# AiX-im/Sample-based-GNN

Measured on AMD Instinct MI355X. Metric: sampled-edges/sec + epoch time, 2-hop GCN on Reddit-shaped graph @1/2/4/8 GPUs, higher is better.
Workload: dtype fp32 (GEMM inputs fp32, split exactly into three bf16 pieces in the kernels, 6 bf16 MFMA products, fp32 accumulate; aggregation fp32)

## Files before the change

sample-based-gnn_amd/csrc/common.hpp:

```cpp
#pragma once
#include <hip/hip_runtime.h>

#include <algorithm>
#include <cstdint>
#include <cstdio>
#include <cstring>
#include <string>
#include <utility>
#include <vector>

#include "nts_hip.h"

namespace nts_hip {

void set_error(const char* fmt, ...);
bool launch_trace();
void launch_trace_sync(const char* file, int line);

#define NTS_HIP_TRY(expr)                                                        \
  do {                                                                           \
    hipError_t _e = (expr);                                                      \
    if (_e != hipSuccess) {                                                      \
      ::nts_hip::set_error("%s:%d: %s failed: %s", __FILE__, __LINE__, #expr,    \
                           hipGetErrorString(_e));                               \
// ... 179 lines not shown
                       __HIP_MEMORY_SCOPE_AGENT);
  return prefix;
}

struct CountArgs {
  const uint64_t* goff;
  const uint32_t* dst;
  const uint32_t* v_in;
  uint32_t v_cap;
  int fanout;
  uint32_t* sizes;
  uint32_t e_cap;
  const uint32_t* omit_map;
  uint32_t omit_key;
  const uint32_t* omit_loc;
  uint32_t* omit_row;
};
int count_scan(nts_hip_ctx* ctx, const CountArgs& ca, uint32_t* co, hipStream_t stream);
size_t count_scan_tmp_elems(uint64_t v_cap);

int radix_sort_pairs(const uint32_t* keys_in, const uint32_t* vals_in, uint32_t* keys_out,
                     uint32_t* vals_out, const uint32_t* n_dev, uint64_t n_cap,
                     uint32_t bits, void* tmp, hipStream_t stream, nts_hip_ctx* ctx = nullptr);
size_t radix_tmp_bytes(uint64_t n_cap);
struct RadixPayload {
  const uint32_t* p1_in = nullptr;
  uint32_t* p1_out = nullptr;
  const uint32_t* p2_in = nullptr;
  uint32_t* p2_out = nullptr;
};
int radix_pass_pairs(const uint32_t* keys_in, const uint32_t* vals_in, uint32_t* keys_out,
                     uint32_t* vals_out, const uint32_t* n_dev, uint64_t n_cap, uint32_t shift,
                     uint32_t dbits, void* tmp, hipStream_t stream, const uint32_t** totals,
                     const RadixPayload& pl = RadixPayload{});
size_t radix_pass_tmp_bytes(uint64_t n_cap);

int sum_splits(hipStream_t st, const float* part, int splits, uint64_t stride, int M, int N,
               float* C, uint64_t ldc);

bool gemm3_nn_ok(int M, int N, int K, const float* A, uint64_t lda);
bool gemm3_tn_ok(int M, int N, int K);
int gemm3_nn(nts_hip_ctx* ctx, bool epi, int M, int N, int K, const float* A, uint64_t lda,
             const uint32_t* amap, const float* B, uint64_t ldb, float* C, uint64_t ldc,
             uint32_t keep_threshold, float scale, uint64_t seed, uint64_t offset);
int gemm3_tn(nts_hip_ctx* ctx, int M, int N, int K, const float* A, uint64_t lda,
             const uint32_t* amap, const float* B, uint64_t ldb, const float* X, uint64_t ldx,
             float bscale, float* C, uint64_t ldc);
bool x3_tn_ok(int M, int N, int K, const float* A, uint64_t lda, const float* B, uint64_t ldb,
              const float* Xm = nullptr, uint64_t ldxm = 0);
bool x3_tn_bm_ok(int M, int N, int K, const float* A, uint64_t lda, const float* B, uint64_t ldb,
                 const float* Xm, uint64_t ldxm);
int x3_tn(nts_hip_ctx* ctx, int M, int N, int K, const float* A, uint64_t lda, const uint32_t* amap,
          const float* B, uint64_t ldb, float* C, uint64_t ldc, const float* Xm = nullptr,
          uint64_t ldxm = 0, float bscale = 1.f);
bool x3_nn_ok(int M, int N, int K, const float* A, uint64_t lda);
bool x3_nn7_ok(int M, int N, int K, const float* A, uint64_t lda);
bool x3_nnk_ok(int M, int N, int K, const float* A, uint64_t lda);
int x3_nn(nts_hip_ctx* ctx, bool epi, int M, int N, int K, const float* A, uint64_t lda,
          const uint32_t* amap, const char* bimg, float* C, uint64_t ldc, uint32_t keep_threshold,
          float scale, uint64_t seed, uint64_t offset);
}
```

sample-based-gnn_amd/csrc/primitives.hip:

```cpp
#include "common.hpp"
#include "radix_tile.hpp"

namespace nts_hip {

constexpr int kScanThreads = 256;
constexpr int kScanItems = 16;
constexpr int kScanTile = kScanThreads * kScanItems;

__device__ __forceinline__ uint32_t pad_idx(uint32_t j) { return j + (j >> 4); }

template <typename T>
__device__ __forceinline__ T wave_incl_scan(T x, int lane) {
#pragma unroll
  for (int o = 1; o < kWave; o <<= 1) {
    T y = __shfl_up(x, o, kWave);
    if (lane >= o) x += y;
  }
  return x;
}

template <typename T>
__device__ __forceinline__ T block_excl_scan(T x, T* wsum , T* total) {
  const int t = threadIdx.x, lane = t & 63, w = t >> 6;
  T inc = wave_incl_scan(x, lane);
// ... 296 lines not shown
  NTS_RET(ensure_scan_state(ctx, scan1_state_elems(n_cap)));
  hipLaunchKernelGGL((k_scan1<false, kScanItems>), dim3((uint32_t)nb), dim3(kScanThreads), 0, stream, in, out,
                     n_dev, n_cap, ctx->scan_state, next_epoch(ctx), scan_ticket(ctx), CountArgs{});
  NTS_LAUNCH_CHECK();
  return NTS_OK;
}

size_t count_scan_tmp_elems(uint64_t v_cap) { return scan_tmp_elems<uint32_t>(v_cap) + 64; }

int count_scan(nts_hip_ctx* ctx, const CountArgs& ca, uint32_t* co, hipStream_t stream) {
  constexpr int kCountItems = 4;
  const uint64_t nb = (uint64_t)ca.v_cap / (kScanThreads * kCountItems) + 1;
  NTS_RET(ensure_scan_state(ctx, (nb + 63) / 64 * 64));
  hipLaunchKernelGGL((k_scan1<true, kCountItems>), dim3((uint32_t)nb), dim3(kScanThreads), 0, stream, nullptr,
                     co, nullptr, (uint64_t)ca.v_cap, ctx->scan_state, next_epoch(ctx), scan_ticket(ctx), ca);
  NTS_LAUNCH_CHECK();
  return NTS_OK;
}

template int scan_exclusive<uint32_t>(const uint32_t*, uint32_t*, const uint32_t*, uint64_t,
                                      uint32_t*, hipStream_t);
template int scan_exclusive<uint64_t>(const uint64_t*, uint64_t*, const uint32_t*, uint64_t,
                                      uint64_t*, hipStream_t);
template size_t scan_tmp_elems<uint32_t>(uint64_t);
template size_t scan_tmp_elems<uint64_t>(uint64_t);

template <int IT>
__global__ __launch_bounds__(kRadixThreads) void k_radix_hist(const uint32_t* __restrict__ keys,
                                                              const uint32_t* n_dev,
                                                              uint64_t n_cap, uint32_t shift,
                                                              uint32_t mask, uint32_t* hist,
                                                              uint32_t nb) {
  __shared__ uint32_t h[kRadixMaxBins];
  const int t = threadIdx.x;
  const uint32_t bins = mask + 1;
  for (uint32_t d = t; d < bins; d += kRadixThreads) h[d] = 0;
  __syncthreads();
  const uint64_t n = n_dev ? (uint64_t)*n_dev : n_cap;
  const uint64_t base = (uint64_t)blockIdx.x * (kRadixThreads * IT);
  if (base >= n) return;
#pragma unroll
  for (int k = 0; k < IT; ++k) {
    const uint64_t i = base + (uint64_t)k * kRadixThreads + t;
    if (i < n) atomicAdd(&h[(keys[i] >> shift) & mask], 1u);
  }
  __syncthreads();
  for (uint32_t d = t; d < bins; d += kRadixThreads) hist[(uint64_t)d * nb + blockIdx.x] = h[d];
}

__global__ __launch_bounds__(kRadixThreads) void k_radix_rowscan(uint32_t* __restrict__ hist,
                                                                 const uint32_t* n_dev, uint64_t n_cap,
                                                                 uint32_t nb, uint32_t tile,
                                                                 uint32_t* __restrict__ totals) {
  __shared__ uint32_t wsum[kRadixThreads / kWave];
  const int t = threadIdx.x;
  const uint64_t n = n_dev ? (uint64_t)*n_dev : n_cap;
  const uint32_t live = (uint32_t)((n + tile - 1) / tile);
  uint32_t* row = hist + (uint64_t)blockIdx.x * nb;
  constexpr int kPer = 4;
  uint32_t carry = 0;
  for (uint32_t c0 = 0; c0 < live; c0 += kRadixThreads * kPer) {
    uint32_t v[kPer], sum = 0;
#pragma unroll
    for (int k = 0; k < kPer; ++k) {
      const uint32_t j = c0 + t * kPer + k;
      v[k] = j < live ? row[j] : 0u;
      sum += v[k];
    }
    uint32_t tot;
    uint32_t run = carry + block_excl_scan(sum, wsum, &tot);
#pragma unroll
    for (int k = 0; k < kPer; ++k) {
      const uint32_t j = c0 + t * kPer + k;
      if (j < live) row[j] = run;
      run += v[k];
    }
    carry += tot;
    __syncthreads();
  }
  if (t == 0) totals[blockIdx.x] = carry;
// ... 42 lines not shown
    }
    __syncthreads();
#pragma unroll
    for (int k = 0; k < IT; ++k)
      if (wbase + (uint64_t)k * kWave + lane < n) sm.sv[loc[k]] = pv[k];
    __syncthreads();
    for (uint32_t i = threadIdx.x; i < cnt; i += kRadixThreads)
      pout[radix_tile_pos(sm, i, sm.sk[i], shift, mask)] = sm.sv[i];
  };
  if (p1_out) payload(p1_in, p1_out);
  if (p2_out) payload(p2_in, p2_out);
}

static size_t radix_tmp_bytes_t(uint64_t n_cap, uint32_t tile) {
  uint64_t nb = (n_cap + tile - 1) / tile;
  if (nb == 0) nb = 1;
  size_t hist = (size_t)kRadixMaxBins * nb + 1;
  size_t elems = 2 * ((n_cap + 63) / 64 * 64) + (hist + 63) / 64 * 64 + kRadixMaxBins + 64;
  return elems * sizeof(uint32_t);
}

size_t radix_tmp_bytes(uint64_t n_cap) { return radix_tmp_bytes_t(n_cap, kRadixTile); }
size_t radix_pass_tmp_bytes(uint64_t n_cap) { return radix_tmp_bytes_t(n_cap, kRadixThreads * kRadixPassItems); }

static uint32_t* radix_totals(void* tmp, uint64_t n_cap, uint32_t tile) {
  const uint32_t nb = ceil_div(n_cap, tile);
  const uint64_t n_al = (n_cap + 63) / 64 * 64;
  return (uint32_t*)tmp + 2 * n_al + ((uint64_t)kRadixMaxBins * nb + 1 + 63) / 64 * 64;
}

template <int IT>
static void radix_pass(const uint32_t* ksrc, const uint32_t* vsrc, uint32_t* kdst, uint32_t* vdst,
                       const uint32_t* n_dev, uint64_t n_cap, uint32_t shift, uint32_t dbits,
                       void* tmp, hipStream_t stream, const RadixPayload& pl = RadixPayload{}) {
  constexpr uint32_t tile = kRadixThreads * IT;
  const uint32_t nb = ceil_div(n_cap, tile);
  const uint64_t n_al = (n_cap + 63) / 64 * 64;
  uint32_t* hist = (uint32_t*)tmp + 2 * n_al;
  uint32_t* totals = radix_totals(tmp, n_cap, tile);
  const uint32_t mask = (1u << dbits) - 1u;
  hipLaunchKernelGGL(k_radix_hist<IT>, dim3(nb), dim3(kRadixThreads), 0, stream, ksrc, n_dev, n_cap,
                     shift, mask, hist, nb);
  hipLaunchKernelGGL(k_radix_rowscan, dim3(mask + 1), dim3(kRadixThreads), 0, stream, hist, n_dev,
                     n_cap, nb, tile, totals);
  hipLaunchKernelGGL(k_radix_scatter<IT>, dim3(nb), dim3(kRadixThreads), 0, stream, ksrc, vsrc, kdst,
                     vdst, n_dev, n_cap, shift, dbits, (const uint32_t*)hist, nb,
                     (const uint32_t*)totals, pl.p1_in, pl.p1_out, pl.p2_in, pl.p2_out);
}

int radix_sort_pairs(const uint32_t* keys_in, const uint32_t* vals_in, uint32_t* keys_out,
                     uint32_t* vals_out, const uint32_t* n_dev, uint64_t n_cap, uint32_t bits,
                     void* tmp, hipStream_t stream, nts_hip_ctx* ctx) {
  (void)ctx;
  if (n_cap == 0) return NTS_OK;
  const uint64_t n_al = (n_cap + 63) / 64 * 64;
  uint32_t* ktmp = (uint32_t*)tmp;
  uint32_t* vtmp = ktmp + n_al;
  if (bits < 1) bits = 1;
  const int npass = (int)((bits + kRadixMaxBits - 1) / kRadixMaxBits);
  const uint32_t dbits = (bits + npass - 1) / npass;
  const uint32_t* ksrc = keys_in;
  const uint32_t* vsrc = vals_in;
  for (int p = 0; p < npass; ++p) {
    bool to_out = ((npass - 1 - p) % 2) == 0;
    uint32_t* kdst = to_out ? keys_out : ktmp;
    uint32_t* vdst = to_out ? vals_out : vtmp;
    radix_pass<kRadixItems>(ksrc, vsrc, kdst, vdst, n_dev, n_cap, dbits * p, dbits, tmp, stream);
    NTS_LAUNCH_CHECK();
    ksrc = kdst;
    vsrc = vdst;
  }
  return NTS_OK;
}

int radix_pass_pairs(const uint32_t* keys_in, const uint32_t* vals_in, uint32_t* keys_out,
                     uint32_t* vals_out, const uint32_t* n_dev, uint64_t n_cap, uint32_t shift,
                     uint32_t dbits, void* tmp, hipStream_t stream, const uint32_t** totals,
                     const RadixPayload& pl) {
  NTS_CHECK_ARG(dbits >= 1 && dbits <= (uint32_t)kRadixMaxBits, "radix digit of 1..9 bits");
  NTS_CHECK_ARG(n_cap > 0, "empty capacity");
  NTS_CHECK_ARG(!(pl.p1_out || pl.p2_out) || !vals_in, "payloads need index values (vals_in NULL)");
  radix_pass<kRadixPassItems>(keys_in, vals_in, keys_out, vals_out, n_dev, n_cap, shift, dbits, tmp,
                              stream, pl);
  NTS_LAUNCH_CHECK();
  *totals = radix_totals(tmp, n_cap, kRadixThreads * kRadixPassItems);
  return NTS_OK;
}

}
```

sample-based-gnn_amd/csrc/radix_tile.hpp:

```cpp
#pragma once
#include "common.hpp"

namespace nts_hip {

constexpr int kRadixThreads = 256;
constexpr int kRadixItems = 16;
constexpr int kRadixTile = kRadixThreads * kRadixItems;
constexpr int kRadixPassItems = 4;
constexpr int kRadixMaxBits = 9;
constexpr int kRadixMaxBins = 1 << kRadixMaxBits;

template <int IT>
struct RadixTileLds {
  uint32_t wh[kRadixThreads / kWave][kRadixMaxBins];
  uint32_t gstart[kRadixMaxBins];
  uint32_t lstart[kRadixMaxBins];
  uint32_t sk[kRadixThreads * IT], sv[kRadixThreads * IT];
  uint32_t wsum[kRadixThreads / kWave];
};

template <int IT, class Pub, class GS>
__device__ __forceinline__ void radix_tile_order(RadixTileLds<IT>& sm, const uint32_t* __restrict__ keys_in,
                                                 const uint32_t* __restrict__ vals_in, uint64_t n,
                                                 uint32_t shift, uint32_t dbits, Pub&& publish,
                                                 GS&& gstart, uint32_t (&loc)[IT]) {
  const int t = threadIdx.x, lane = t & 63, w = t >> 6;
  const uint64_t base = (uint64_t)blockIdx.x * (kRadixThreads * IT);
  const uint32_t mask = (1u << dbits) - 1u, bins = mask + 1;
  for (uint32_t d = t; d < bins; d += kRadixThreads)
#pragma unroll
    for (int ww = 0; ww < kRadixThreads / kWave; ++ww) sm.wh[ww][d] = 0;
  __syncthreads();
  const uint64_t lt_mask = (lane == 0) ? 0ull : (~0ull >> (64 - lane));
  const uint64_t wbase = base + (uint64_t)w * (IT * kWave);
  uint32_t key[IT], val[IT], rank[IT];
#pragma unroll
  for (int k = 0; k < IT; ++k) {
    const uint64_t i = wbase + (uint64_t)k * kWave + lane;
    const bool valid = i < n;
    key[k] = valid ? keys_in[i] : 0u;
    val[k] = valid ? (vals_in ? vals_in[i] : (uint32_t)i) : 0u;
  }
#pragma unroll
  for (int k = 0; k < IT; ++k) {
    const bool valid = wbase + (uint64_t)k * kWave + lane < n;
    const uint32_t d = (key[k] >> shift) & mask;
    uint64_t peers = __ballot(valid);
    for (uint32_t b = 0; b < dbits; ++b) {
      const bool bit = (d >> b) & 1u;
      const uint64_t m = __ballot(bit);
      peers &= bit ? m : ~m;
    }
// ... 66 lines not shown
```

sample-based-gnn_amd/csrc/sampler.hip:

```cpp
#include "mfma_lds.hpp"

#include <type_traits>

namespace nts_hip {

constexpr int kSelThreads = 256;
constexpr int kSelWaves = kSelThreads / kWave;
constexpr int kSetCap = 1024;

__device__ __forceinline__ uint32_t philox_word(uint64_t seed, uint32_t dst, uint32_t layer,
                                                uint64_t batch_seq, uint32_t idx) {
  uint4 c = make_uint4(idx >> 2, dst, layer, (uint32_t)batch_seq);
  uint2 k = make_uint2((uint32_t)seed, (uint32_t)(seed >> 32) ^ (uint32_t)(batch_seq >> 32));
  uint4 r = philox4x32_10(c, k);
  uint32_t j = idx & 3u;
  return j == 0 ? r.x : (j == 1 ? r.y : (j == 2 ? r.z : r.w));
}

struct Draw {
  uint32_t range, thr, scaling, past;
  bool lemire;
  __device__ __forceinline__ void init(uint32_t r, bool lem) {
    range = r;
    lemire = lem;
    thr = (0u - r) % r;
    scaling = 0xFFFFFFFFu / r;
    past = r * scaling;
  }
  __device__ __forceinline__ bool apply(uint32_t x, uint32_t& v) const {
    if (lemire) {
      uint64_t m = (uint64_t)x * range;
      v = (uint32_t)(m >> 32);
      return (uint32_t)m >= thr;
    }
    v = x / scaling;
    return x < past;
  }
};

struct SelectArgs {
  const uint64_t* goff;
  const uint32_t* grows;
  const uint32_t* dst;
  const uint32_t* co;
  uint32_t* sizes;
  uint32_t* ans;
  uint32_t* edst;
  uint8_t* marks;
  uint32_t e_cap;
  int fanout;
  uint32_t layer;
  uint64_t batch_seq;
  uint64_t seed;
};

__device__ __forceinline__ void copy_all(const SelectArgs& a, uint32_t i, uint64_t beg,
                                         uint32_t deg, uint32_t c, int lane) {
  for (uint32_t k = lane; k < deg; k += kWave) {
    uint32_t g = a.grows[beg + k];
    a.ans[c + k] = g;
    a.edst[c + k] = i;
    a.marks[g] = 1;
  }
}

template <typename WordFn>
__device__ __forceinline__ uint32_t select_distinct(const SelectArgs& a, uint32_t i,
                                                    uint64_t beg, uint32_t deg, uint32_t need,
                                                    uint32_t c, int lane, uint32_t* set,
                                                    const Draw& dr, WordFn word) {
  const uint64_t lt_mask = (lane == 0) ? 0ull : (~0ull >> (64 - lane));
  uint32_t count = 0, consumed = 0;
  while (count < need) {
    const uint32_t remaining = need - count;
    const int R = remaining <= 12 ? 16 : (remaining <= 28 ? 32 : 64);
    uint32_t val = 0;
    bool ok = false;
    if (lane < R) ok = dr.apply(word(consumed + lane), val);
    bool dup = false;
    for (uint32_t j = 0; j < count; ++j) dup |= (set[j] == val);
    const uint64_t okmask = __ballot(ok);
// ... 75 lines not shown
      dup |= (j < lane) && ((okmask >> j) & 1ull) && (vj == val);
    }
    const uint64_t newmask = __ballot(ok && !dup);
    uint64_t take = newmask;
    if ((uint32_t)__popcll(newmask) >= remaining) {
      uint64_t m = newmask;
      for (uint32_t t = 1; t < remaining; ++t) m &= m - 1;
      const int last = __ffsll((long long)m) - 1;
      take = newmask & ((last == 63) ? ~0ull : ((2ull << last) - 1ull));
      consumed += (uint32_t)last + 1u;
    } else {
      consumed += (uint32_t)kWave;
    }
    if ((take >> lane) & 1ull) {
      hset_put(hset, mask, val);
      out[count + (uint32_t)__popcll(take & lt_mask)] = val;
    }
    count += (uint32_t)__popcll(take);
    __syncthreads();
  }
  for (uint32_t k = lane; k < cap; k += kWave) hset[k] = 0u;
  __syncthreads();
  return consumed;
}

__global__ __launch_bounds__(kWave) void k_select_philox_big(SelectArgs a, uint32_t cap) {
  extern __shared__ uint32_t hset[];
  const int lane = threadIdx.x;
  for (uint32_t k = lane; k < cap; k += kWave) hset[k] = 0u;
  __syncthreads();
  const uint32_t v = a.sizes[0];
  for (uint32_t i = blockIdx.x; i < v; i += gridDim.x) {
    const uint32_t d = a.dst[i];
    const uint64_t beg = a.goff[d];
    const uint32_t deg = (uint32_t)(a.goff[d + 1] - beg);
    const uint32_t c = a.co[i];
    const uint32_t n = a.co[i + 1] - c;
    if (c + n > a.e_cap) continue;
    if (n == deg) {
      copy_all(a, i, beg, deg, c, lane);
      continue;
    }
    if (n == 0) continue;
    const uint64_t seed = a.seed, bs = a.batch_seq;
    const uint32_t layer = a.layer;
    select_distinct_hashed(n, hset, cap, lane, deg, (0u - deg) % deg, true, a.ans + c,
                           [&](uint32_t j) { return philox_word(seed, d, layer, bs, j); });
    for (uint32_t k = lane; k < n; k += kWave) {
      const uint32_t g = a.grows[beg + a.ans[c + k]];
      a.ans[c + k] = g;
      a.edst[c + k] = i;
      a.marks[g] = 1;
    }
  }
}

__global__ __launch_bounds__(kSelThreads) void k_select_philox(SelectArgs a) {
  __shared__ uint32_t sets[kSelWaves][kSetCap];
  const int lane = threadIdx.x & 63, w = threadIdx.x >> 6;
  const uint32_t v = a.sizes[0];
  uint32_t* set = sets[w];
  const uint32_t nw = gridDim.x * kSelWaves;
  for (uint32_t i = blockIdx.x * kSelWaves + w; i < v; i += nw) {
    const uint32_t d = a.dst[i];
    const uint64_t beg = a.goff[d];
    const uint32_t deg = (uint32_t)(a.goff[d + 1] - beg);
    const uint32_t c = a.co[i];
    const uint32_t n = a.co[i + 1] - c;
    if (c + n > a.e_cap) continue;
    if (n == deg) {
      copy_all(a, i, beg, deg, c, lane);
    } else if (n > 0) {
      Draw dr;
      dr.init(deg, true);
      const uint64_t seed = a.seed;
      const uint32_t layer = a.layer;
      const uint64_t bs = a.batch_seq;
      select_distinct(a, i, beg, deg, n, c, lane, set, dr, [&](uint32_t j) {
        return philox_word(seed, d, layer, bs, j);
      });
    }
  }
}

constexpr int kGrp = 16;
constexpr int kGrpPerWave = kWave / kGrp;

template <int J>
struct GrpDupScan {
  static __device__ __forceinline__ void run(bool& dup, uint32_t val, int gl, uint32_t okm) {
    const uint32_t vj = (uint32_t)__builtin_amdgcn_update_dpp(0, (int)val, 0x150 + J, 0xF, 0xF, false);
    dup |= (J < gl) && ((okm >> J) & 1u) && (vj == val);
    GrpDupScan<J + 1>::run(dup, val, gl, okm);
  }
};
template <>
struct GrpDupScan<kGrp> {
  static __device__ __forceinline__ void run(bool&, uint32_t, int, uint32_t) {}
};

__global__ __launch_bounds__(kSelThreads) void k_select_philox_g16(SelectArgs a) {
  __shared__ uint32_t sets[kSelWaves * kGrpPerWave][kGrp];
  const int lane = threadIdx.x & 63, w = threadIdx.x >> 6;
  const int gl = lane & (kGrp - 1), grp = lane >> 4;
  const int gib = w * kGrpPerWave + grp;
  uint32_t* set = sets[gib];
  const uint32_t gshift = kGrp * grp;
  const uint32_t lt16 = (1u << gl) - 1u;
  const uint32_t v = a.sizes[0];
  const uint32_t ng = gridDim.x * kSelWaves * kGrpPerWave;
  for (uint32_t i = blockIdx.x * kSelWaves * kGrpPerWave + gib; i < v; i += ng) {
    const uint32_t d = a.dst[i];
    const uint64_t beg = a.goff[d];
    const uint32_t deg = (uint32_t)(a.goff[d + 1] - beg);
    const uint32_t c = a.co[i];
    const uint32_t n = a.co[i + 1] - c;
    if (c + n > a.e_cap) continue;
    if (n == deg) {
      for (uint32_t k = gl; k < deg; k += kGrp) {
        const uint32_t g = a.grows[beg + k];
        a.ans[c + k] = g;
        a.edst[c + k] = i;
        a.marks[g] = 1;
      }
      continue;
    }
    if (n == 0) continue;
    Draw dr;
    dr.init(deg, true);
    uint32_t count = 0, consumed = 0;
    while (count < n) {
      const uint32_t remaining = n - count;
      uint32_t val = 0;
      const bool ok = dr.apply(philox_word(a.seed, d, a.layer, a.batch_seq, consumed + gl), val);
      bool dup = false;
      for (uint32_t j = 0; j < count; ++j) dup |= (set[j] == val);
      const uint32_t okm = (uint32_t)(__ballot(ok) >> gshift) & 0xFFFFu;
      GrpDupScan<0>::run(dup, val, gl, okm);
      const bool isnew = ok && !dup;
      const uint32_t newm = (uint32_t)(__ballot(isnew) >> gshift) & 0xFFFFu;
      uint32_t take = newm;
      if ((uint32_t)__popc(newm) >= remaining) {
        uint32_t m = newm;
        for (uint32_t t = 1; t < remaining; ++t) m &= m - 1;
        const int last = __ffs(m) - 1;
// ... 908 lines not shown
  const uint32_t words[4] = {m.x, m.y, m.z, m.w};
  const uint64_t v0 = tid * 16;
#pragma unroll
  for (int q = 0; q < 4; ++q) {
#pragma unroll
    for (int b = 0; b < 4; ++b) {
      if ((words[q] >> (8 * b)) & 0xffu) {
        const uint64_t vtx = v0 + q * 4 + b;
        if (vtx < n_vertices && pos < s_cap) {
          source[pos] = (uint32_t)vtx;
          src_index[vtx] = pos;
        }
        ++pos;
      }
    }
  }
}


struct RelabelArgs {
  const uint32_t* ans;
  const uint32_t* edst;
  const uint32_t* dst;
  const uint32_t* src_index;
  const uint32_t* out_deg;
  const uint32_t* in_deg;
  const uint32_t* co;
  const uint32_t* sizes;
  int weight_type;
  uint32_t* ri;
  float* wf;
  uint32_t* up_cnt;
  uint32_t* pub;
};

__device__ __forceinline__ void publish_sizes(const uint32_t* sizes, uint32_t* pub) {
  if (pub && blockIdx.x == 0 && threadIdx.x < 4) pub[threadIdx.x] = sizes[threadIdx.x];
}

__device__ __forceinline__ uint32_t relabel_one(const RelabelArgs& a, uint32_t k) {
  const uint32_t g = a.ans[k];
  const uint32_t r = a.src_index[g];
  a.ri[k] = r;
  if (a.up_cnt) {
    atomicAdd(a.up_cnt + r, 1u);
  } else if (a.weight_type != NTS_WEIGHT_NONE) {
    const uint32_t dg = a.dst[a.edst[k]];
    const uint32_t ind = a.in_deg[dg];
    float w = norm_degree(a.out_deg[g], ind);
    if (a.weight_type == NTS_WEIGHT_MEAN) w = mean_weight(w, ind);
    if (a.weight_type == NTS_WEIGHT_MEAN_SAMPLED) w = w / (float)(a.co[a.edst[k] + 1] - a.co[a.edst[k]]);
    a.wf[k] = w;
  }
  return r;
}

__global__ void k_relabel(RelabelArgs a) {
  publish_sizes(a.sizes, a.pub);
  const uint32_t e = a.sizes[1];
  for (uint32_t k = blockIdx.x * blockDim.x + threadIdx.x; k < e; k += gridDim.x * blockDim.x)
    relabel_one(a, k);
}

__global__ void k_up_weight(const uint32_t* __restrict__ ri, const uint32_t* __restrict__ edst,
                            const uint32_t* __restrict__ co, const uint32_t* __restrict__ cnt,
                            const uint32_t* sizes, int weight_type, float* __restrict__ wf,
                            uint32_t* pub) {
  publish_sizes(sizes, pub);
  const uint32_t e = sizes[1];
  for (uint32_t k = blockIdx.x * blockDim.x + threadIdx.x; k < e; k += gridDim.x * blockDim.x) {
    const uint32_t d = edst[k];
    const uint32_t ind = co[d + 1] - co[d];
    float w = norm_degree(cnt[ri[k]], ind);
    if (weight_type == NTS_WEIGHT_MEAN || weight_type == NTS_WEIGHT_MEAN_SAMPLED)
      w = w / (float)ind;
    wf[k] = w;
  }
}

__global__ void k_mark_dst(const uint32_t* __restrict__ dst, const uint32_t* sizes,
                           uint8_t* __restrict__ marks) {
  const uint32_t v = sizes[0];
  for (uint32_t d = blockIdx.x * blockDim.x + threadIdx.x; d < v; d += gridDim.x * blockDim.x)
    marks[dst[d]] = 1;
}
__global__ void k_dst_local(const uint32_t* __restrict__ dst, const uint32_t* __restrict__ src_index,
                            const uint32_t* sizes, uint32_t* __restrict__ dl) {
  const uint32_t v = sizes[0];
  for (uint32_t d = blockIdx.x * blockDim.x + threadIdx.x; d < v; d += gridDim.x * blockDim.x)
    dl[d] = src_index[dst[d]];
}

constexpr int kCsrBucketThreads = 1024;
constexpr int kCsrBucketWaves = kCsrBucketThreads / kWave;
constexpr int kCsrBucketIt = 4;

template <int L>
__global__ __launch_bounds__(kCsrBucketThreads) void k_csr_bucket(
    const uint32_t* __restrict__ skey, const uint32_t* __restrict__ seid,
    const uint32_t* __restrict__ totals, const uint32_t* __restrict__ sdst,
    const uint32_t* __restrict__ swf, const uint32_t* sizes, uint32_t* __restrict__ ro,
    uint32_t* __restrict__ ci, float* __restrict__ wb, uint32_t* __restrict__ ceid, uint32_t* pub) {
  constexpr uint32_t R = 1u << L, RPT = R > kCsrBucketThreads ? R / kCsrBucketThreads : 1;
  __shared__ uint32_t wh[kCsrBucketWaves][R];
  __shared__ uint32_t wsum[kCsrBucketWaves];
  publish_sizes(sizes, pub);
  const int t = threadIdx.x, lane = t & 63, w = t >> 6;
  const uint32_t b = blockIdx.x, s = sizes[2], r0 = b << L;
  if (r0 > s) return;
  uint32_t part = 0;
  for (uint32_t i = t; i < b; i += kCsrBucketThreads) part += totals[i];
#pragma unroll
  for (int o = 32; o >= 1; o >>= 1) part += __shfl_xor(part, o, kWave);
  if (lane == 0) wsum[w] = part;
  for (uint32_t d = t; d < R; d += kCsrBucketThreads)
#pragma unroll
    for (int ww = 0; ww < kCsrBucketWaves; ++ww) wh[ww][d] = 0;
  __syncthreads();
  uint32_t bstart = 0;
#pragma unroll
  for (int ww = 0; ww < kCsrBucketWaves; ++ww) bstart += wsum[ww];
  const uint32_t cnt = totals[b];
  const uint32_t q0 = (uint32_t)((uint64_t)cnt * w / kCsrBucketWaves);
// ... 347 lines not shown
  uint32_t* t_swf = t_sdst + sort_p / 2;
  uint32_t* t_up = t_sdst + sort_p;
  uint32_t* t_mt = t_up + up_n;
  void* t_sort = (void*)(t_mt + mt_n);

  const uint32_t gv = std::max(1u, std::min(ceil_div(o->v_cap, 256), kMaxGrid));
  const uint32_t ge = std::max(1u, std::min(ceil_div(o->e_cap, 256), kMaxGrid));

  {
    CountArgs ca;
    ca.goff = g->column_offset;
    ca.dst = o->destination;
    ca.v_in = o->v_size;
    ca.v_cap = o->v_cap;
    ca.fanout = fanout;
    ca.sizes = o->sizes;
    ca.e_cap = o->e_cap;
    ca.omit_map = o->omit_map;
    ca.omit_key = o->omit_key;
    ca.omit_loc = o->omit_loc;
    ca.omit_row = o->omit_row;
    NTS_RET(count_scan(ctx, ca, o->column_offset, st));
  }

  SelectArgs a;
  a.goff = g->column_offset;
  a.grows = g->row_indices;
  a.dst = o->destination;
  a.co = o->column_offset;
  a.sizes = o->sizes;
  a.ans = o->sample_ans;
  a.edst = o->edge_dst;
  a.marks = ctx->marks;
  a.e_cap = o->e_cap;
  a.fanout = fanout;
  a.layer = (uint32_t)layer;
  a.batch_seq = batch_seq;
  a.seed = ctx->seed;
  if (rng_mode == NTS_RNG_PHILOX) {
    if (fanout >= 0 && fanout <= kGrp) {
      const uint32_t gs =
          std::max(1u, std::min(ceil_div(o->v_cap, kSelWaves * kGrpPerWave), 4096u));
      hipLaunchKernelGGL(k_select_philox_g16, dim3(gs), dim3(kSelThreads), 0, st, a);
    } else if (fanout < 0 || fanout <= kSetCap) {
      const uint32_t gs = std::max(1u, std::min(ceil_div(o->v_cap, kSelWaves), 4096u));
      hipLaunchKernelGGL(k_select_philox, dim3(gs), dim3(kSelThreads), 0, st, a);
    } else {
      uint32_t cap = 1;
      while (cap < 2u * (uint32_t)fanout) cap <<= 1;
      const size_t lds = (size_t)cap * sizeof(uint32_t);
      NTS_HIP_TRY(hipFuncSetAttribute(reinterpret_cast<const void*>(&k_select_philox_big),
                                      hipFuncAttributeMaxDynamicSharedMemorySize, (int)lds));
      const uint32_t gs = std::max(1u, std::min(o->v_cap, 2048u));
      hipLaunchKernelGGL(k_select_philox_big, dim3(gs), dim3(kWave), lds, st, a, cap);
    }
  } else {
    const int lem = rng_mode == NTS_RNG_MT19937_LEMIRE ? 1 : 0;
    constexpr int mt_dbg = 0;
    uint4* info = reinterpret_cast<uint4*>(t_mt);
    uint64_t gen_hi = 0;
    uint32_t seq = 0;
    NTS_RET(mt_ring_prepare(ctx, w_cap, st, &gen_hi, &seq));
    if (mt_chunked) {
      uint32_t* base = t_mt + mt_info_n;
      float2* cstat = reinterpret_cast<float2*>(base + mt_base_n);
      uint2* win = reinterpret_cast<uint2*>(base + mt_base_n + mt_stat_n);
// ... 30 lines not shown
      else if (fanout <= 16) NTS_RET(run(I16{}, I16{}));
      else if (fanout <= 25) NTS_RET(run(std::integral_constant<int, 25>{}, I32{}));
      else NTS_RET(run(I32{}, I32{}));
      NTS_LAUNCH_CHECK();
      NTS_RET(mt_ring_finish(ctx, st));
      const uint32_t gs = std::max(1u, std::min(ceil_div(o->v_cap, kSelWaves * kGrpPerWave), 4096u));
      hipLaunchKernelGGL(k_mt_rows, dim3(gs), dim3(kSelThreads), 0, st, a);
      NTS_LAUNCH_CHECK();
      goto frontier;
    }
    hipLaunchKernelGGL(k_mt_prep, dim3(gv), dim3(256), 0, st, g->column_offset, o->destination,
                       o->column_offset, o->sizes, o->e_cap, lem, info, nullptr, nullptr, 1u,
                       nullptr, nullptr);
    NTS_LAUNCH_CHECK();
    const MtChunked whole{ctx->mt_ring, nullptr, gen_hi, nullptr, nullptr, ctx->mt_done, seq,
                          o->sizes + 3};
    if (fanout >= 0 && fanout <= 16)
      hipLaunchKernelGGL((k_mt_serial<16, false>), dim3(1), dim3(kWave), 0, st, info, o->sizes,
                         o->sample_ans, ctx->mt_state, lem, mt_dbg, whole);
    else if (fanout >= 0 && fanout <= 32)
      hipLaunchKernelGGL((k_mt_serial<32, false>), dim3(1), dim3(kWave), 0, st, info, o->sizes,
                         o->sample_ans, ctx->mt_state, lem, mt_dbg, whole);
    else
      hipLaunchKernelGGL((k_mt_serial<64, false>), dim3(1), dim3(kWave), 0, st, info, o->sizes,
                         o->sample_ans, ctx->mt_state, lem, mt_dbg, whole);
    NTS_LAUNCH_CHECK();
    NTS_RET(mt_ring_finish(ctx, st));
    const uint32_t gs = std::max(1u, std::min(ceil_div(o->v_cap, kSelWaves * kGrpPerWave), 4096u));
    hipLaunchKernelGGL(k_mt_rows, dim3(gs), dim3(kSelThreads), 0, st, a);
  }
  NTS_LAUNCH_CHECK();

frontier:
  if (o->dst_local_id) {
    hipLaunchKernelGGL(k_mark_dst, dim3(gv), dim3(256), 0, st, o->destination, o->sizes,
                       ctx->marks);
    NTS_LAUNCH_CHECK();
  }

  constexpr uint32_t kMarkFusedMaxTiles = 256;
  if (nblk_marks <= kMarkFusedMaxTiles) {
    NTS_RET(ensure_scan_state(ctx, scan1_state_elems((uint64_t)nblk_marks * 4096)));
    hipLaunchKernelGGL(k_mark_fused, dim3(nblk_marks), dim3(kMarkThreads), 0, st, ctx->marks,
                       nblk_marks, V, o->s_cap, o->source, ctx->src_index, o->sizes,
                       ctx->scan_state, scan_next_epoch(ctx), scan_ticket(ctx));
    NTS_LAUNCH_CHECK();
  } else {
    hipLaunchKernelGGL(k_mark_count, dim3(nblk_marks), dim3(kMarkThreads), 0, st, ctx->marks,
                       t_blk);
    NTS_LAUNCH_CHECK();
    if (nblk_marks <= kMarkDirectTiles) {
      hipLaunchKernelGGL(k_mark_write<true>, dim3(nblk_marks), dim3(kMarkThreads), 0, st,
                         ctx->marks, t_blk, nblk_marks, V, o->s_cap, o->source, ctx->src_index,
                         o->sizes);
    } else {
      NTS_RET(scan_exclusive<uint32_t>(t_blk, t_blk, nullptr, nblk_marks, t_scan_blk, st));
      hipLaunchKernelGGL(k_mark_write<false>, dim3(nblk_marks), dim3(kMarkThreads), 0, st,
                         ctx->marks, t_blk, nblk_marks, V, o->s_cap, o->source, ctx->src_index,
                         o->sizes);
    }
    NTS_LAUNCH_CHECK();
  }

  if (o->dst_local_id) {
    hipLaunchKernelGGL(k_dst_local, dim3(gv), dim3(256), 0, st, o->destination, ctx->src_index,
                       o->sizes, o->dst_local_id);
    NTS_LAUNCH_CHECK();
  }

  RelabelArgs ra{o->sample_ans,      o->edge_dst, o->destination, ctx->src_index,
                 g->out_degree,      g->in_degree, o->column_offset, o->sizes,
                 weight_type,        o->row_indices, o->edge_weight_forward,
                 up ? t_up : nullptr, (up || csr) ? nullptr : o->sizes_host};
  if (up) NTS_HIP_TRY(hipMemsetAsync(t_up, 0, up_n * sizeof(uint32_t), st));
  hipLaunchKernelGGL(k_relabel, dim3(ge), dim3(256), 0, st, ra);
  NTS_LAUNCH_CHECK();
  if (up) {
    hipLaunchKernelGGL(k_up_weight, dim3(ge), dim3(256), 0, st, o->row_indices, o->edge_dst,
                       o->column_offset, t_up, o->sizes, weight_type, o->edge_weight_forward,
                       csr ? nullptr : o->sizes_host);
    NTS_LAUNCH_CHECK();
  }

  if (csr) {
    const uint32_t bits = ceil_log2((uint64_t)o->s_cap + 1);
    if (bits >= 11 && bits <= 19) {
      const uint32_t H = std::min(9u, bits - 6), L = bits - H;
      const uint32_t* totals = nullptr;
      const bool wpl = weight_type != NTS_WEIGHT_NONE && o->edge_weight_backward;
      RadixPayload pl;
      pl.p1_in = o->edge_dst;
      pl.p1_out = t_sdst;
      if (wpl) {
        pl.p2_in = reinterpret_cast<const uint32_t*>(o->edge_weight_forward);
        pl.p2_out = t_swf;
      }
      NTS_RET(radix_pass_pairs(o->row_indices, nullptr, t_skey, o->csr_edge_id ? t_seid : nullptr,
                               o->sizes + 1, o->e_cap, L, H, t_sort, st, &totals, pl));
      const uint32_t* swf = wpl ? t_swf : nullptr;
#define NTS_CSR_BUCKET(LL)                                                                        \
  hipLaunchKernelGGL(k_csr_bucket<LL>, dim3(1u << H), dim3(kCsrBucketThreads), 0, st, t_skey,   \
                     t_seid, totals, t_sdst, swf, o->sizes, o->row_offset, o->column_indices,   \
                     o->edge_weight_backward, o->csr_edge_id, o->sizes_host)
      switch (L) {
        case 6: NTS_CSR_BUCKET(6); break;
        case 7: NTS_CSR_BUCKET(7); break;
        case 8: NTS_CSR_BUCKET(8); break;
        case 9: NTS_CSR_BUCKET(9); break;
        default: NTS_CSR_BUCKET(10); break;
      }
#undef NTS_CSR_BUCKET
      NTS_LAUNCH_CHECK();
      return NTS_OK;
    }
    NTS_RET(radix_sort_pairs(o->row_indices, nullptr, t_skey, t_seid, o->sizes + 1, o->e_cap,
                             bits, t_sort, st, ctx));
    hipLaunchKernelGGL(k_csr_finalize, dim3(ge), dim3(256), 0, st, t_skey, t_seid, o->edge_dst,
                       weight_type == NTS_WEIGHT_NONE ? nullptr : o->edge_weight_forward,
                       o->sizes, o->row_offset, o->column_indices, o->edge_weight_backward,
                       o->csr_edge_id, o->sizes_host);
    NTS_LAUNCH_CHECK();
  }
  return NTS_OK;
}

extern "C" int nts_hip_mt_budget_scale(nts_hip_ctx* ctx, double scale) {
  NTS_CHECK_ARG(ctx, "ctx is NULL");
  NTS_CHECK_ARG(scale > 0.0 && scale < 1e6, "scale must be > 0");
  ctx->mt_budget_scale = scale;
  return NTS_OK;
}
// ... 17 lines not shown
```

Baseline: 1.899 billion.

## Fuse radix histogram into relabel and fold dst marking/local-id into sampler

Result: no change. 1.895 billion (-0.2%).

```diff
diff --git a/sample-based-gnn_amd/csrc/common.hpp b/sample-based-gnn_amd/csrc/common.hpp
--- a/sample-based-gnn_amd/csrc/common.hpp
+++ b/sample-based-gnn_amd/csrc/common.hpp
@@ -235,7 +235,8 @@
 int radix_pass_pairs(const uint32_t* keys_in, const uint32_t* vals_in, uint32_t* keys_out,
                      uint32_t* vals_out, const uint32_t* n_dev, uint64_t n_cap, uint32_t shift,
                      uint32_t dbits, void* tmp, hipStream_t stream, const uint32_t** totals,
-                     const RadixPayload& pl = RadixPayload{});
+                     const RadixPayload& pl = RadixPayload{}, bool counted = false);
+uint32_t* radix_pass_counts(void* tmp, uint64_t n_cap, uint32_t* nb);
 size_t radix_pass_tmp_bytes(uint64_t n_cap);
 
 int sum_splits(hipStream_t st, const float* part, int splits, uint64_t stride, int M, int N,
diff --git a/sample-based-gnn_amd/csrc/primitives.hip b/sample-based-gnn_amd/csrc/primitives.hip
--- a/sample-based-gnn_amd/csrc/primitives.hip
+++ b/sample-based-gnn_amd/csrc/primitives.hip
@@ -352,20 +352,8 @@
                                                               uint32_t mask, uint32_t* hist,
                                                               uint32_t nb) {
   __shared__ uint32_t h[kRadixMaxBins];
-  const int t = threadIdx.x;
-  const uint32_t bins = mask + 1;
-  for (uint32_t d = t; d < bins; d += kRadixThreads) h[d] = 0;
-  __syncthreads();
   const uint64_t n = n_dev ? (uint64_t)*n_dev : n_cap;
-  const uint64_t base = (uint64_t)blockIdx.x * (kRadixThreads * IT);
-  if (base >= n) return;
-#pragma unroll
-  for (int k = 0; k < IT; ++k) {
-    const uint64_t i = base + (uint64_t)k * kRadixThreads + t;
-    if (i < n) atomicAdd(&h[(keys[i] >> shift) & mask], 1u);
-  }
-  __syncthreads();
-  for (uint32_t d = t; d < bins; d += kRadixThreads) hist[(uint64_t)d * nb + blockIdx.x] = h[d];
+  radix_tile_hist<IT>(h, n, shift, mask, hist, nb, [&](int, uint64_t i) { return keys[i]; });
 }
 
 __global__ __launch_bounds__(kRadixThreads) void k_radix_rowscan(uint32_t* __restrict__ hist,
@@ -474,15 +462,17 @@
 template <int IT>
 static void radix_pass(const uint32_t* ksrc, const uint32_t* vsrc, uint32_t* kdst, uint32_t* vdst,
                        const uint32_t* n_dev, uint64_t n_cap, uint32_t shift, uint32_t dbits,
-                       void* tmp, hipStream_t stream, const RadixPayload& pl = RadixPayload{}) {
+                       void* tmp, hipStream_t stream, const RadixPayload& pl = RadixPayload{},
+                       bool counted = false) {
   constexpr uint32_t tile = kRadixThreads * IT;
   const uint32_t nb = ceil_div(n_cap, tile);
   const uint64_t n_al = (n_cap + 63) / 64 * 64;
   uint32_t* hist = (uint32_t*)tmp + 2 * n_al;
   uint32_t* totals = radix_totals(tmp, n_cap, tile);
   const uint32_t mask = (1u << dbits) - 1u;
-  hipLaunchKernelGGL(k_radix_hist<IT>, dim3(nb), dim3(kRadixThreads), 0, stream, ksrc, n_dev, n_cap,
-                     shift, mask, hist, nb);
+  if (!counted)
+    hipLaunchKernelGGL(k_radix_hist<IT>, dim3(nb), dim3(kRadixThreads), 0, stream, ksrc, n_dev,
+                       n_cap, shift, mask, hist, nb);
   hipLaunchKernelGGL(k_radix_rowscan, dim3(mask + 1), dim3(kRadixThreads), 0, stream, hist, n_dev,
                      n_cap, nb, tile, totals);
   hipLaunchKernelGGL(k_radix_scatter<IT>, dim3(nb), dim3(kRadixThreads), 0, stream, ksrc, vsrc, kdst,
@@ -515,15 +505,20 @@
   return NTS_OK;
 }
 
+uint32_t* radix_pass_counts(void* tmp, uint64_t n_cap, uint32_t* nb) {
+  *nb = ceil_div(n_cap, (uint32_t)(kRadixThreads * kRadixPassItems));
+  return (uint32_t*)tmp + 2 * ((n_cap + 63) / 64 * 64);
+}
+
 int radix_pass_pairs(const uint32_t* keys_in, const uint32_t* vals_in, uint32_t* keys_out,
                      uint32_t* vals_out, const uint32_t* n_dev, uint64_t n_cap, uint32_t shift,
                      uint32_t dbits, void* tmp, hipStream_t stream, const uint32_t** totals,
-                     const RadixPayload& pl) {
+                     const RadixPayload& pl, bool counted) {
   NTS_CHECK_ARG(dbits >= 1 && dbits <= (uint32_t)kRadixMaxBits, "radix digit of 1..9 bits");
   NTS_CHECK_ARG(n_cap > 0, "empty capacity");
   NTS_CHECK_ARG(!(pl.p1_out || pl.p2_out) || !vals_in, "payloads need index values (vals_in NULL)");
   radix_pass<kRadixPassItems>(keys_in, vals_in, keys_out, vals_out, n_dev, n_cap, shift, dbits, tmp,
-                              stream, pl);
+                              stream, pl, counted);
   NTS_LAUNCH_CHECK();
   *totals = radix_totals(tmp, n_cap, kRadixThreads * kRadixPassItems);
   return NTS_OK;
diff --git a/sample-based-gnn_amd/csrc/radix_tile.hpp b/sample-based-gnn_amd/csrc/radix_tile.hpp
--- a/sample-based-gnn_amd/csrc/radix_tile.hpp
+++ b/sample-based-gnn_amd/csrc/radix_tile.hpp
@@ -18,6 +18,24 @@
   uint32_t sk[kRadixThreads * IT], sv[kRadixThreads * IT];
   uint32_t wsum[kRadixThreads / kWave];
 };
+
+template <int IT, class KeyFn>
+__device__ __forceinline__ void radix_tile_hist(uint32_t* h, uint64_t n, uint32_t shift, uint32_t mask,
+                                                uint32_t* __restrict__ hist, uint32_t nb, KeyFn&& key) {
+  const int t = threadIdx.x;
+  const uint32_t bins = mask + 1;
+  for (uint32_t d = t; d < bins; d += kRadixThreads) h[d] = 0;
+  __syncthreads();
+  const uint64_t base = (uint64_t)blockIdx.x * (kRadixThreads * IT);
+  if (base >= n) return;
+#pragma unroll
+  for (int k = 0; k < IT; ++k) {
+    const uint64_t i = base + (uint64_t)k * kRadixThreads + t;
+    if (i < n) atomicAdd(&h[(key(k, i) >> shift) & mask], 1u);
+  }
+  __syncthreads();
+  for (uint32_t d = t; d < bins; d += kRadixThreads) hist[(uint64_t)d * nb + blockIdx.x] = h[d];
+}
 
 template <int IT, class Pub, class GS>
 __device__ __forceinline__ void radix_tile_order(RadixTileLds<IT>& sm, const uint32_t* __restrict__ keys_in,
diff --git a/sample-based-gnn_amd/csrc/sampler.hip b/sample-based-gnn_amd/csrc/sampler.hip
--- a/sample-based-gnn_amd/csrc/sampler.hip
+++ b/sample-based-gnn_amd/csrc/sampler.hip
@@ -1,4 +1,5 @@
 #include "mfma_lds.hpp"
+#include "radix_tile.hpp"
 
 #include <type_traits>
 
@@ -47,6 +48,7 @@
   uint32_t* ans;
   uint32_t* edst;
   uint8_t* marks;
+  uint8_t* dmarks;
   uint32_t e_cap;
   int fanout;
   uint32_t layer;
@@ -188,6 +190,7 @@
   const uint32_t v = a.sizes[0];
   for (uint32_t i = blockIdx.x; i < v; i += gridDim.x) {
     const uint32_t d = a.dst[i];
+    if (a.dmarks && lane == 0) a.dmarks[d] = 1;
     const uint64_t beg = a.goff[d];
     const uint32_t deg = (uint32_t)(a.goff[d + 1] - beg);
     const uint32_t c = a.co[i];
@@ -219,6 +222,7 @@
   const uint32_t nw = gridDim.x * kSelWaves;
   for (uint32_t i = blockIdx.x * kSelWaves + w; i < v; i += nw) {
     const uint32_t d = a.dst[i];
+    if (a.dmarks && lane == 0) a.dmarks[d] = 1;
     const uint64_t beg = a.goff[d];
     const uint32_t deg = (uint32_t)(a.goff[d + 1] - beg);
     const uint32_t c = a.co[i];
@@ -267,6 +271,7 @@
   const uint32_t ng = gridDim.x * kSelWaves * kGrpPerWave;
   for (uint32_t i = blockIdx.x * kSelWaves * kGrpPerWave + gib; i < v; i += ng) {
     const uint32_t d = a.dst[i];
+    if (a.dmarks && gl == 0) a.dmarks[d] = 1;
     const uint64_t beg = a.goff[d];
     const uint32_t deg = (uint32_t)(a.goff[d + 1] - beg);
     const uint32_t c = a.co[i];
@@ -1241,7 +1246,15 @@
   float* wf;
   uint32_t* up_cnt;
   uint32_t* pub;
+  uint32_t* dl;
 };
+
+__device__ __forceinline__ void dst_local(const RelabelArgs& a) {
+  if (!a.dl) return;
+  const uint32_t v = a.sizes[0];
+  for (uint32_t d = blockIdx.x * blockDim.x + threadIdx.x; d < v; d += gridDim.x * blockDim.x)
+    a.dl[d] = a.src_index[a.dst[d]];
+}
 
 __device__ __forceinline__ void publish_sizes(const uint32_t* sizes, uint32_t* pub) {
   if (pub && blockIdx.x == 0 && threadIdx.x < 4) pub[threadIdx.x] = sizes[threadIdx.x];
@@ -1266,9 +1279,55 @@
 
 __global__ void k_relabel(RelabelArgs a) {
   publish_sizes(a.sizes, a.pub);
+  dst_local(a);
   const uint32_t e = a.sizes[1];
   for (uint32_t k = blockIdx.x * blockDim.x + threadIdx.x; k < e; k += gridDim.x * blockDim.x)
     relabel_one(a, k);
+}
+
+template <int IT>
+__global__ __launch_bounds__(kRadixThreads) void k_relabel_hist(RelabelArgs a, uint32_t shift,
+                                                                uint32_t mask, uint32_t* hist,
+                                                                uint32_t nb) {
+  __shared__ uint32_t h[kRadixMaxBins];
+  dst_local(a);
+  const uint32_t e = a.sizes[1];
+  const uint64_t base = (uint64_t)blockIdx.x * (kRadixThreads * IT);
+  const bool wts = a.weight_type != NTS_WEIGHT_NONE;
+  uint32_t r[IT];
+  if (base < e) {
+    uint32_t g[IT], ed[IT], dg[IT], od[IT], ind[IT], cn[IT];
+    bool ok[IT];
+#pragma unroll
+    for (int k = 0; k < IT; ++k) {
+      const uint64_t i = base + (uint64_t)k * kRadixThreads + threadIdx.x;
+      ok[k] = i < e;
+      g[k] = ok[k] ? a.ans[i] : 0u;
+      ed[k] = ok[k] && wts ? a.edst[i] : 0u;
+    }
+#pragma unroll
+    for (int k = 0; k < IT; ++k) {
+      r[k] = ok[k] ? a.src_index[g[k]] : 0u;
+      od[k] = ok[k] && wts ? a.out_deg[g[k]] : 0u;
+      dg[k] = ok[k] && wts ? a.dst[ed[k]] : 0u;
+      cn[k] = ok[k] && a.weight_type == NTS_WEIGHT_MEAN_SAMPLED ? a.co[ed[k] + 1] - a.co[ed[k]] : 1u;
+    }
+#pragma unroll
+    for (int k = 0; k < IT; ++k) ind[k] = ok[k] && wts ? a.in_deg[dg[k]] : 0u;
+#pragma unroll
+    for (int k = 0; k < IT; ++k) {
+      if (!ok[k]) continue;
+      const uint64_t i = base + (uint64_t)k * kRadixThreads + threadIdx.x;
+      a.ri[i] = r[k];
+      if (wts) {
+        float w = norm_degree(od[k], ind[k]);
+        if (a.weight_type == NTS_WEIGHT_MEAN) w = mean_weight(w, ind[k]);
+        if (a.weight_type == NTS_WEIGHT_MEAN_SAMPLED) w = w / (float)cn[k];
+        a.wf[i] = w;
+      }
+    }
+  }
+  radix_tile_hist<IT>(h, e, shift, mask, hist, nb, [&](int k, uint64_t) { return r[k]; });
 }
 
 __global__ void k_up_weight(const uint32_t* __restrict__ ri, const uint32_t* __restrict__ edst,
@@ -1292,12 +1351,6 @@
   const uint32_t v = sizes[0];
   for (uint32_t d = blockIdx.x * blockDim.x + threadIdx.x; d < v; d += gridDim.x * blockDim.x)
     marks[dst[d]] = 1;
-}
-__global__ void k_dst_local(const uint32_t* __restrict__ dst, const uint32_t* __restrict__ src_index,
-                            const uint32_t* sizes, uint32_t* __restrict__ dl) {
-  const uint32_t v = sizes[0];
-  for (uint32_t d = blockIdx.x * blockDim.x + threadIdx.x; d < v; d += gridDim.x * blockDim.x)
-    dl[d] = src_index[dst[d]];
 }
 
 constexpr int kCsrBucketThreads = 1024;
@@ -1711,6 +1764,7 @@
   a.ans = o->sample_ans;
   a.edst = o->edge_dst;
   a.marks = ctx->marks;
+  a.dmarks = o->dst_local_id && rng_mode == NTS_RNG_PHILOX ? ctx->marks : nullptr;
   a.e_cap = o->e_cap;
   a.fanout = fanout;
   a.layer = (uint32_t)layer;
@@ -1807,7 +1861,7 @@
   NTS_LAUNCH_CHECK();
 
 frontier:
-  if (o->dst_local_id) {
+  if (o->dst_local_id && !a.dmarks) {
     hipLaunchKernelGGL(k_mark_dst, dim3(gv), dim3(256), 0, st, o->destination, o->sizes,
                        ctx->marks);
     NTS_LAUNCH_CHECK();
@@ -1837,18 +1891,23 @@
     NTS_LAUNCH_CHECK();
   }
 
-  if (o->dst_local_id) {
-    hipLaunchKernelGGL(k_dst_local, dim3(gv), dim3(256), 0, st, o->destination, ctx->src_index,
-                       o->sizes, o->dst_local_id);
-    NTS_LAUNCH_CHECK();
-  }
-
+  const uint32_t key_bits = ceil_log2((uint64_t)o->s_cap + 1);
+  const bool csr_bucket = csr && key_bits >= 11 && key_bits <= 19;
+  const uint32_t key_hi = std::min(9u, key_bits - 6), key_lo = key_bits - key_hi;
+  const bool relabel_counts = csr_bucket && !up && o->e_cap > 0;
   RelabelArgs ra{o->sample_ans,      o->edge_dst, o->destination, ctx->src_index,
                  g->out_degree,      g->in_degree, o->column_offset, o->sizes,
                  weight_type,        o->row_indices, o->edge_weight_forward,
-                 up ? t_up : nullptr, (up || csr) ? nullptr : o->sizes_host};
+                 up ? t_up : nullptr, (up || csr) ? nullptr : o->sizes_host, o->dst_local_id};
   if (up) NTS_HIP_TRY(hipMemsetAsync(t_up, 0, up_n * sizeof(uint32_t), st));
-  hipLaunchKernelGGL(k_relabel, dim3(ge), dim3(256), 0, st, ra);
+  if (relabel_counts) {
+    uint32_t nb = 0;
+    uint32_t* counts = radix_pass_counts(t_sort, o->e_cap, &nb);
+    hipLaunchKernelGGL(k_relabel_hist<kRadixPassItems>, dim3(nb), dim3(kRadixThreads), 0, st, ra,
+                       key_lo, (1u << key_hi) - 1u, counts, nb);
+  } else {
+    hipLaunchKernelGGL(k_relabel, dim3(ge), dim3(256), 0, st, ra);
+  }
   NTS_LAUNCH_CHECK();
   if (up) {
     hipLaunchKernelGGL(k_up_weight, dim3(ge), dim3(256), 0, st, o->row_indices, o->edge_dst,
@@ -1858,9 +1917,9 @@
   }
 
   if (csr) {
-    const uint32_t bits = ceil_log2((uint64_t)o->s_cap + 1);
-    if (bits >= 11 && bits <= 19) {
-      const uint32_t H = std::min(9u, bits - 6), L = bits - H;
+    const uint32_t bits = key_bits;
+    if (csr_bucket) {
+      const uint32_t H = key_hi, L = key_lo;
       const uint32_t* totals = nullptr;
       const bool wpl = weight_type != NTS_WEIGHT_NONE && o->edge_weight_backward;
       RadixPayload pl;
@@ -1871,7 +1930,8 @@
         pl.p2_out = t_swf;
       }
       NTS_RET(radix_pass_pairs(o->row_indices, nullptr, t_skey, o->csr_edge_id ? t_seid : nullptr,
-                               o->sizes + 1, o->e_cap, L, H, t_sort, st, &totals, pl));
+                               o->sizes + 1, o->e_cap, L, H, t_sort, st, &totals, pl,
+                               relabel_counts));
       const uint32_t* swf = wpl ? t_swf : nullptr;
 #define NTS_CSR_BUCKET(LL)                                                                        \
   hipLaunchKernelGGL(k_csr_bucket<LL>, dim3(1u << H), dim3(kCsrBucketThreads), 0, st, t_skey,   \
```
